# resemble-ai/flowhigh

Hardware: NVIDIA B200
Metric: 48kHz audio-sec/sec (whole job) (higher is better)
Workload: dtype fp16

## Files before the change

flowhigh_b200/_lib.py:

```python
from __future__ import annotations

import ctypes as C
import os
from typing import Optional

from .build import lib_path

_i, _i64, _f, _p = C.c_int, C.c_int64, C.c_float, C.c_void_p


class TcConvArgs(C.Structure):
    _fields_ = [
        ("a", _p), ("a_batch", _i64), ("a_chunk", _i64), ("a_row0", _i),
        ("w", _p), ("bias", _p), ("res", _p), ("out", _p),
        ("out_batch", _i64), ("out_chunk", _i64), ("out_row", _i64),
        ("res_batch", _i64), ("res_chunk", _i64), ("res_row", _i64),
        ("out_is_16", _i), ("res_is_16", _i),
        ("alpha", _f), ("beta_res", _f),
        ("accumulate", _i), ("geglu", _i),
        ("B", _i), ("L", _i), ("Cin", _i), ("Cout", _i),
        ("ntaps", _i), ("P", _i),
        ("tap_off", C.POINTER(_i)),
        ("bn", _i),
        ("fp16", _i),
# ... 30 lines not shown
    "fh_dwconv_gelu_res_f32": (_i, [_p, _p, _p, _p, _i, _i, _i, _i, _p]),
    "fh_dwconv_f32": (_i, [_p, _p, _p, _p, _i, _i, _i, _i, _p]),
    "fh_layernorm_f32": (_i, [_p, _p, _p, _p, _i, _i64, _i, _i, _f, _p]),
    "fh_gelu_f32": (_i, [_p, _p, _i, _i64, _i, _i, _p]),
    "fh_rmsnorm_f32": (_i, [_p, _p, _p, _p, _i, _i64, _i, _i, _p]),
    "fh_qknorm_rope_f32": (_i, [_p, _p, _p, _p, _p, _p, _p, _i, _i, _i, _i, _p]),
    "fh_attention_f32": (_i, [_p, _p, _p, _p, _i, _i64, _i, _i, _i, _i, _f, _p]),
    "fh_qknorm_rope_split": (_i, [_p, _p, _p, _p, _p, _p, _p, _p, _p, _i, _i, _i, _i, _f, _i, _p]),
    "fh_attention_tc": (_i, [_p, _p, _p, _p, _p, _p, _i, _i64, _i, _i, _i, _i, _i, _p]),
    "fh_attention_tc5_operand_elems": (_i64, [_i, _i, _i, _i]),
    "fh_qknorm_rope_tiles": (_i, [_p, _p, _p, _p, _p, _p, _p, _i, _i, _i, _i, _f, _i, _p]),
    "fh_attention_tc5": (_i, [_p, _p, _p, _p, _i, _i64, _i, _i, _i, _i, _i, _p]),
    "fh_geglu_f32": (_i, [_p, _p, _i, _i64, _i, _i, _i, _p]),
    "fh_axpby_f32": (_i, [_p, _p, _f, _f, _p, _i64, _p]),
    "fh_rk_lincomb_f32": (_i, [_p, _p, _i64, _i, C.POINTER(_f), _p, _i64, _p]),
    "fh_rk_scaled_sumsq_f32": (_i, [_p, _p, _p, _f, _f, _i, _i64, _p, _p]),
    "fh_broadcast_row_f32": (_i, [_p, _p, _i64, _i, _p]),
    "fh_mel_cutoff_f32": (_i, [_p, _p, _i, _i, _i, _f, _p]),
    "fh_mel_splice_f32": (_i, [_p, _p, _p, _p, _i, _i, _i, _p]),
    "fh_conv1d_taps_f32": (_i, [_p, _p, _p, _p, _p, _f, _f, _i, _p, _i, _i, _i, _i, _i, _i, _p]),
    "fh_snake_aa_f32": (_i, [_p, _p, _p, _p, _p, _i, _i, _i, _p]),
    "fh_convpost_tanh_f32": (_i, [_p, _p, _f, _p, _i, _i, _i, _p]),
    "fh_transpose_f32": (_i, [_p, _p, _i, _i, _i, _p]),
    "fh_cast_f32_16": (_i, [_p, _p, _i64, _i, _p]),
    "fh_cast_f32_16_split": (_i, [_p, _p, _i64, _i, _i64, _i64, _i, _i, _p]),
    "fh_sum_cast_f32": (_i, [_p, _p, _p, _p, _p, _p, _i64, _i, _p]),
    "fh_tc_conv": (_i, [C.POINTER(TcConvArgs), _p]),
    "fh_tc_packed_weight_bytes": (_i64, [_i, _i, _i, _i, _i]),
    "fh_to_chunked_16": (_i, [_p, _i64, _i64, _i64, _p, _i64, _i64, _i, _i, _i, _i, _i, _p]),
    "fh_to_chunked_16_split": (_i, [_p, _i64, _i64, _i64, _p, _i64, _i64, _i, _i, _i, _i, _i, _p]),
    "fh_snake_aa_chunked_split": (_i, [_p, _p, _p, _p, _p, _i64, _i64, _i64, _i, _i, _i, _i, _p]),
    "fh_snake_aa_chunked": (_i, [_p, _p, _p, _p, _p, _i64, _i64, _i, _i, _i, _i, _i, _p]),
    "fh_snake_aa_chunked_h": (_i, [_p, _p, _p, _p, _p, _i64, _i64, _i, _i, _i, _i, _p]),
    "fh_snakepost_convpost_tanh": (_i, [_p, _i64, _i64, _i, _p, _p, _p, _p, _f, _p, _i, _i, _i, _p]),
    "fh_convpost_tanh_chunked": (_i, [_p, _i64, _i64, _i, _p, _f, _p, _i, _i, _i, _p]),
}

_lib: Optional[C.CDLL] = None


class FlowHighNativeError(RuntimeError):
    pass


def load(build_if_missing: bool = True) -> C.CDLL:
    global _lib
    if _lib is not None:
        return _lib
    path = lib_path()
    if build_if_missing and os.environ.get("FLOWHIGH_B200_NO_BUILD") != "1":
        try:
            from .build import build
            path = build()
        except Exception as e:
            if not os.path.exists(path):
                raise FlowHighNativeError(f"libflowhigh_b200.so is missing and cannot be built: {e}") from e
    if not os.path.exists(path):
        raise FlowHighNativeError(
            f"{path} not found: run `python -m flowhigh_b200.build` (nvcc, sm_100a). There is no fallback path.")
    lib = C.CDLL(path)
    for name, (res, args) in SIGNATURES.items():
        fn = getattr(lib, name)
        fn.restype = res
        fn.argtypes = args
    _lib = lib
    return lib
# ... 16 lines not shown
```

flowhigh_b200/csrc/snake_mma.cuh:

```cuda
#pragma once
#include <cuda_fp16.h>
#include "snake_worker.cuh"
#ifndef FH_SNAKE_K8
#define FH_SNAKE_K8 1
#endif

namespace fh {

template <int NB>
struct SnakeMmaGeom {
  static constexpr int kWarps = 4;
  static constexpr int kSeg = 8 * NB;
  static constexpr int kWarpRows = 2 * kSeg;
  static constexpr int kRows = kWarps * kWarpRows;
  static constexpr int kHalo = 8;
  static constexpr int kXRows = kRows + 2 * kHalo;
  static constexpr int kXBytes = kXRows * 32;
  static constexpr int kWarpYBytes = kWarpRows * 16;
  static constexpr int smem_bytes(bool in16, bool split_out = false, int wbuf = 2) {
    return wbuf * (in16 ? kXBytes / 2 : kXBytes) + (split_out ? 4 : 2) * kWarps * kWarpYBytes + 128;
  }
};

__device__ __forceinline__ uint32_t sm_pack(float lo, float hi) {
// ... 213 lines not shown
      }
    }
  }
  if (edge) {
    __syncwarp();
    for (int w = lane; w < 48; w += 32) {
      const int c = w & 7, o = w >> 3;
      const int qq = o < 3 ? o : L - 6 + o;
      if (qq >= q0 && qq < q0 + G::kWarpRows && qq < L && (o < 3 || qq >= 3)) {
        const int cc = ch * 8 + c;
        const float alv = 2.0f * __ldg(sn_a + cc), hib = 0.5f * __ldg(sn_inv_b + cc);
        float acc = hib;
        for (int k = 0; k < 12; ++k) {
          const int m = min(max(2 * qq + k - 5, 0), 2 * L - 1);
          const int ihi = (m + 5) >> 1;
          float u = 0.f;
          for (int t6 = 0; t6 < 6; ++t6) {
            const int i = ihi - t6;
            const int ic = min(max(i, 0), L - 1);
            const int xi = (ic - q0 + G::kHalo) * 8 + c;
            const float xv = IN16 ? __half2float(reinterpret_cast<const __half*>(xw)[xi]) : xw[xi];
            u = fmaf(2.0f * __ldg(sn_filt + (m + 5 - 2 * i)), xv, u);
          }
          acc = fmaf(__ldg(sn_filt + k), u - hib * __cosf(alv * u), acc);
        }
        const __half hv = __float2half_rn(acc);
        *reinterpret_cast<__half*>(yt + (size_t)(qq - q0) * 16 + 2 * c) = hv;
        if (SPLIT_OUT) *reinterpret_cast<__half*>(yt_lo + (size_t)(qq - q0) * 16 + 2 * c) = __float2half_rn(acc - __half2float(hv));
      }
    }
  }
}

template <bool SPLIT_X, bool SPLIT_F, int NB, bool IN16 = false, bool SPLIT_OUT = false, int WBUF = 2>
__device__ __forceinline__ void snake_mma_cta(const SnakeParams& S, unsigned char* smem, int tid, int cta, int nctas) {
  using G = SnakeMmaGeom<NB>;
  const int lane = tid & 31, warp = tid >> 5;
  constexpr int kXB = IN16 ? G::kXBytes / 2 : G::kXBytes;
  float* xs0 = reinterpret_cast<float*>(smem);
  float* xs1 = reinterpret_cast<float*>(smem + (WBUF - 1) * kXB);
  constexpr int kImg = SPLIT_OUT ? 2 : 1;
  unsigned char* ys0 = smem + WBUF * kXB + warp * 2 * kImg * G::kWarpYBytes;
  unsigned char* ctl = smem + WBUF * kXB + 2 * kImg * G::kWarps * G::kWarpYBytes;
  const uint32_t bar0 = sw_u32(ctl);
  int* released = reinterpret_cast<int*>(ctl + 16);
  float* s_taps = reinterpret_cast<float*>(ctl + 32);
  if (tid == 0) {
    asm volatile("mbarrier.init.shared::cta.b64 [%0], 1;" ::"r"(bar0) : "memory");
    asm volatile("mbarrier.init.shared::cta.b64 [%0], 1;" ::"r"(bar0 + 8) : "memory");
    asm volatile("fence.mbarrier_init.release.cluster;" ::: "memory");
    released[0] = released[1] = 0;
  }
  if (tid < 4) snake_mma_make_taps<SPLIT_F>(S.filt, s_taps, tid);
  for (int i = tid; i < WBUF * kXB / 16; i += 32 * G::kWarps) reinterpret_cast<float4*>(smem)[i] = make_float4(0.f, 0.f, 0.f, 0.f);
  asm volatile("fence.proxy.async.shared::cta;" ::: "memory");
  __syncthreads();
  const int rows_per_chunk = (int)(S.chunk_stride >> 3);
  const int d_tile = nctas % S.ntile, d_rest = nctas / S.ntile;
  const int d_ch = d_rest % S.nchunk, d_b = d_rest / S.nchunk;
  auto advance = [&](int& tile, int& ch, int& b) {
    tile += d_tile;
    ch += d_ch;
    b += d_b;
    if (tile >= S.ntile) tile -= S.ntile, ++ch;
    if (ch >= S.nchunk) ch -= S.nchunk, ++b;
  };
  auto issue = [&](int tile, int ch, int b, int buf) {
    const int r_first = S.row0 + tile * G::kRows - G::kHalo;
    int nrows = rows_per_chunk - r_first;
    nrows = nrows < G::kXRows ? nrows : G::kXRows;
    const long long eoff = (long long)b * S.batch_stride + (long long)ch * S.chunk_stride + (long long)r_first * 8;
    const void* src = IN16 ? (const void*)((const unsigned short*)S.x + eoff) : (const void*)(S.x + eoff);
    const uint32_t bytes = (uint32_t)nrows * (IN16 ? 16u : 32u);
    const uint32_t bar = bar0 + 8 * buf;
    asm volatile("mbarrier.arrive.expect_tx.shared::cta.b64 _, [%0], %1;" ::"r"(bar), "r"(bytes) : "memory");
    asm volatile("cp.async.bulk.shared::cluster.global.mbarrier::complete_tx::bytes [%0], [%1], %2, [%3];" ::"r"(
                     sw_u32(buf ? xs1 : xs0)),
                 "l"(src), "r"(bytes), "r"(bar)
                 : "memory");
  };

  SnakeFrags F;
  snake_mma_frags<IN16>(s_taps, lane, F);
  Guard16 guard;
  int item = cta;
  int tile = item % S.ntile, ch = (item / S.ntile) % S.nchunk, b = (item / S.ntile) / S.nchunk;
  int tile_f = tile, ch_f = ch, b_f = b;
  if (tid == 0 && item < S.total) issue(tile, ch, b, 0);
  advance(tile_f, ch_f, b_f);
  if (WBUF == 2) {
    if (tid == 0 && item + nctas < S.total) issue(tile_f, ch_f, b_f, 1);
    advance(tile_f, ch_f, b_f);
  }
  int buf = 0, ybuf = 0;
  uint32_t ph0 = 0, ph1 = 0;
  const int ssA = warp * G::kWarpRows;
  for (; item < S.total; item += nctas, advance(tile, ch, b), advance(tile_f, ch_f, b_f)) {
    const int qt = tile * G::kRows;
    const bool edge = (tile == 0) || (qt + G::kRows + G::kHalo > S.L);
    const bool active = qt + ssA < S.L;
    sw_mbar_wait(bar0 + 8 * buf, buf ? ph1 : ph0);
    if (buf) ph1 ^= 1; else ph0 ^= 1;
    float* xt = buf ? xs1 : xs0;
    unsigned char* yt = ys0 + (size_t)ybuf * kImg * G::kWarpYBytes;
    if (active) {
      float* xw = reinterpret_cast<float*>(reinterpret_cast<unsigned char*>(xt) + (size_t)ssA * (IN16 ? 16 : 32));
      snake_mma_unit<SPLIT_X, SPLIT_F, NB, IN16, SPLIT_OUT>(F, xw, yt, qt + ssA, S.L, ch, S.a, S.inv_b, S.filt, edge, -ssA,
                                                            G::kXRows - ssA, lane, guard, yt + G::kWarpYBytes);
    }
    asm volatile("fence.proxy.async.shared::cta;" ::: "memory");
    if (lane == 0) asm volatile("cp.async.bulk.wait_group.read 0;" ::: "memory");
    __syncwarp();
    if (lane == 0) {
      if (active) {
        const int nrows = min(G::kWarpRows, S.L - qt - ssA);
        const unsigned short* dst = (const unsigned short*)S.y + (long long)b * S.y_batch_stride +
                                    (long long)ch * S.chunk_stride + (long long)(S.row0 + qt + ssA) * 8;
        asm volatile("cp.async.bulk.global.shared::cta.bulk_group [%0], [%1], %2;" ::"l"(dst), "r"(sw_u32(yt)),
                     "r"((uint32_t)nrows * 16u)
                     : "memory");
        if (SPLIT_OUT)
          asm volatile("cp.async.bulk.global.shared::cta.bulk_group [%0], [%1], %2;" ::"l"(dst + S.lo_offset),
                       "r"(sw_u32(yt + G::kWarpYBytes)), "r"((uint32_t)nrows * 16u)
                       : "memory");
        asm volatile("cp.async.bulk.commit_group;" ::: "memory");
      }
      __threadfence_block();
      if (atomicAdd(&released[buf], 1) == G::kWarps - 1) {
        released[buf] = 0;
        __threadfence_block();
        if (item + WBUF * nctas < S.total) {
          asm volatile("fence.proxy.async.shared::cta;" ::: "memory");
          issue(tile_f, ch_f, b_f, buf);
        }
      }
    }
    if (WBUF == 2) buf ^= 1;
    ybuf ^= 1;
  }
  if (lane == 0) asm volatile("cp.async.bulk.wait_group.read 0;" ::: "memory");
  guard.commit(S.status, 1);
}

}
```

flowhigh_b200/csrc/snake_worker.cuh:

```cuda
#pragma once
#include "common.cuh"

namespace fh {

struct SnakeParams {
  const float* x;
  void* y;
  const float* a;
  const float* inv_b;
  const float* filt;
  long long batch_stride, chunk_stride;
  long long y_batch_stride;
  long long lo_offset;
  int row0, nchunk, L, ntile, total;
  int fp16;
  unsigned int* status;
};

template <int R>
struct SnakeGeom {
  static constexpr int kRows = R * 32;
  static constexpr int kXRows = kRows + 10;
  static constexpr int kXBytes = kXRows * 32;
  static constexpr int kYBytes = kRows * 16;
  static constexpr int kSmemBytes = ((2 * kXBytes + kYBytes + 16 + 127) / 128) * 128;
};

__device__ __forceinline__ float2 sw_ffma2(float2 a, float2 b, float2 c) {
  unsigned long long ra = *reinterpret_cast<unsigned long long*>(&a), rb = *reinterpret_cast<unsigned long long*>(&b),
                     rc = *reinterpret_cast<unsigned long long*>(&c), rd;
  asm("fma.rn.f32x2 %0, %1, %2, %3;" : "=l"(rd) : "l"(ra), "l"(rb), "l"(rc));
  return *reinterpret_cast<float2*>(&rd);
}
__device__ __forceinline__ float2 sw_fmul2(float2 a, float2 b) {
  unsigned long long ra = *reinterpret_cast<unsigned long long*>(&a), rb = *reinterpret_cast<unsigned long long*>(&b), rd;
  asm("mul.rn.f32x2 %0, %1, %2;" : "=l"(rd) : "l"(ra), "l"(rb));
  return *reinterpret_cast<float2*>(&rd);
}
__device__ __forceinline__ uint32_t sw_u32(const void* p) { return (uint32_t)__cvta_generic_to_shared(p); }
__device__ __forceinline__ void sw_mbar_wait(uint32_t bar, uint32_t parity) {
  uint32_t ok = 0;
  const long long t0 = clock64();
  while (!ok) {
    asm volatile(
        "{\n\t.reg .pred p;\n\t"
        "mbarrier.try_wait.parity.shared::cta.b64 p, [%1], %2, %3;\n\t"
        "selp.b32 %0, 1, 0, p;\n\t}"
        : "=r"(ok)
        : "r"(bar), "r"(parity), "r"(2000u)
// ... 155 lines not shown
```

flowhigh_b200/csrc/vocoder_tc.cu:

```cuda
#include <stdlib.h>
#include "common.cuh"
#include "snake_worker.cuh"
#include "snake_mma.cuh"

namespace {

constexpr int PR = 17;

template <int OUT_KIND, bool BULK_OUT>
__global__ void __launch_bounds__(128, 4) snake_aa_chunked_tma_kernel(const __grid_constant__ fh::SnakeParams S) {
  extern __shared__ __align__(128) unsigned char snake_smem[];
  fh::snake_worker<OUT_KIND, BULK_OUT, PR>(S, snake_smem, threadIdx.x, blockIdx.x, gridDim.x, 0);
}

template <int MODE, int NB, int MINB, bool IN16, bool SPLIT_OUT, int WBUF>
__global__ void __launch_bounds__(128, MINB) snake_aa_mma_kernel(const __grid_constant__ fh::SnakeParams S) {
  extern __shared__ __align__(128) unsigned char snake_smem[];
  fh::snake_mma_cta<(MODE & 1) != 0, (MODE & 2) != 0, NB, IN16, SPLIT_OUT, WBUF>(S, snake_smem, threadIdx.x, blockIdx.x,
                                                                                 gridDim.x);
}

template <int MODE, int NB, int MINB, bool IN16 = false, bool SPLIT_OUT = false, int WBUF = 2>
void launch_snake_mma(fh::SnakeParams sp, int B, int C, int L, int sms, cudaStream_t stream) {
  using G = fh::SnakeMmaGeom<NB>;
  static int smem_set[64] = {0};
  fh::ensure_dyn_smem(snake_aa_mma_kernel<MODE, NB, MINB, IN16, SPLIT_OUT, WBUF>, G::smem_bytes(IN16, SPLIT_OUT, WBUF), smem_set);
  sp.ntile = (L + G::kRows - 1) / G::kRows;
  const long long total = (long long)sp.ntile * (C / 8) * B;
  sp.total = (int)total;
  const int grid = (int)(total < (long long)sms * MINB ? total : (long long)sms * MINB);
  snake_aa_mma_kernel<MODE, NB, MINB, IN16, SPLIT_OUT, WBUF><<<grid, 128, G::smem_bytes(IN16, SPLIT_OUT, WBUF), stream>>>(sp);
}

constexpr int kCpT = 256;
__global__ void __launch_bounds__(kCpT) convpost_tanh_chunked_kernel(const float* __restrict__ x, long long batch_stride,
                                                                     long long chunk_stride, int row0,
                                                                     const float* __restrict__ w, float bias,
                                                                     float* __restrict__ y, int C, int L) {
  extern __shared__ __align__(16) float cp_smem[];
  const int nchunk = C >> 3;
  float* s_w = cp_smem;
  float* tile = cp_smem + ((C * 7 + 3) & ~3);
  const int b = blockIdx.y, t0 = blockIdx.x * kCpT;
  for (int i = threadIdx.x; i < C * 7; i += kCpT) s_w[i] = __ldg(w + i);
  const float* xb = x + (long long)b * batch_stride;
  const int rows = kCpT + 6;
  for (int i = threadIdx.x; i < nchunk * rows * 2; i += kCpT) {
    const int h = i & 1, r = (i >> 1) % rows, ch = (i >> 1) / rows;
    const int t = t0 - 3 + r;
    float4 v = make_float4(0.f, 0.f, 0.f, 0.f);
    if (t >= 0 && t < L) v = __ldg(reinterpret_cast<const float4*>(xb + (long long)ch * chunk_stride + (long long)(row0 + t) * 8) + h);
    reinterpret_cast<float4*>(tile)[i] = v;
  }
  __syncthreads();
  const int t = t0 + threadIdx.x;
  if (t >= L) return;
  float acc = bias;
  for (int ch = 0; ch < nchunk; ++ch) {
    const float* tp = tile + ((size_t)ch * rows + threadIdx.x) * 8;
    const float* wp = s_w + ch * 56;
#pragma unroll
    for (int j = 0; j < 7; ++j) {
      const float4 v0 = *reinterpret_cast<const float4*>(tp + j * 8), v1 = *reinterpret_cast<const float4*>(tp + j * 8 + 4);
      acc = fmaf(wp[j], v0.x, acc);
// ... 113 lines not shown
    for (int r = 0; r < 10; ++r) {
      const float4 v0 = *reinterpret_cast<const float4*>(tp + sp_row_off(o + r));
      const float4 v1 = *reinterpret_cast<const float4*>(tp + sp_row_off(o + r) + 16);
      const float v[8] = {v0.x, v0.y, v0.z, v0.w, v1.x, v1.y, v1.z, v1.w};
#pragma unroll
      for (int oo = 0; oo < 4; ++oo) {
        const int j = r - oo;
        if (j >= 0 && j < 7) {
#pragma unroll
          for (int c = 0; c < 8; ++c) acc[oo] = fmaf(wr[c * 7 + j], v[c], acc[oo]);
        }
      }
    }
  }
  float* yp = y + (long long)b * L + t0 + o;
  if (t0 + o + 3 < L && ((((long long)b * L + t0 + o) & 3) == 0)) {
    *reinterpret_cast<float4*>(yp) = make_float4(tanhf(acc[0]), tanhf(acc[1]), tanhf(acc[2]), tanhf(acc[3]));
  } else {
#pragma unroll
    for (int oo = 0; oo < 4; ++oo)
      if (t0 + o + oo < L) yp[oo] = tanhf(acc[oo]);
  }
}

}

extern "C" __attribute__((visibility("default"))) int fh_snake_aa_chunked(
    const float* x, void* y, const float* a, const float* inv_b, const float* filt, int64_t batch_stride,
    int64_t chunk_stride, int row0, int B, int C, int L, int out_kind, void* stream) {
  FH_REQUIRE(B > 0 && C > 0 && (C % 8) == 0 && L > 0, FH_ERR_BAD_SHAPE, "fh_snake_aa_chunked: C must be a multiple of 8");
  FH_REQUIRE(out_kind >= 0 && out_kind <= 2, FH_ERR_BAD_SHAPE, "fh_snake_aa_chunked: out_kind must be 0 (fp32), 1 (bf16), 2 (fp16)");
  FH_REQUIRE(((uintptr_t)x % 16) == 0 && (batch_stride % 8) == 0 && (chunk_stride % 8) == 0, FH_ERR_BAD_ALIGN,
             "fh_snake_aa_chunked: x must be 16-byte aligned and strides multiples of 8");
  static int mma_mode = -2;
  if (mma_mode == -2) {
    const char* e = getenv("FH_SNAKE_MMA");
    mma_mode = e ? atoi(e) : 0;
    if (mma_mode < -1 || mma_mode > 3) mma_mode = 0;
  }
  const bool use_mma = out_kind == 2 && mma_mode >= 0 && row0 >= fh::SnakeMmaGeom<8>::kHalo;
  constexpr int kTileRows = fh::SnakeGeom<PR>::kRows;
  const int ntile = (L + kTileRows - 1) / kTileRows;
  const long long total = (long long)ntile * (C / 8) * B;
  FH_REQUIRE(total <= 2147483647LL && row0 >= 5, FH_ERR_BAD_SHAPE, "fh_snake_aa_chunked: needs a left halo of >= 5 rows");
  const int sms = fh::dev_sms();
  static int per_sm = 0;
  if (!per_sm) {
    const char* e = getenv("FH_SNAKE_CTAS_PER_SM");
    per_sm = e ? atoi(e) : 4;
    if (per_sm < 1 || per_sm > 4) per_sm = 4;
  }
  const int grid = (int)(total < (long long)sms * per_sm ? total : (long long)sms * per_sm);
  static int bulk = -1;
  if (bulk < 0) {
    const char* e = getenv("FH_SNAKE_BULK");
    bulk = e ? atoi(e) : 1;
  }
  fh::SnakeParams sp;
  sp.x = x, sp.y = y, sp.a = a, sp.inv_b = inv_b, sp.filt = filt;
  sp.batch_stride = batch_stride, sp.chunk_stride = chunk_stride, sp.y_batch_stride = batch_stride, sp.lo_offset = 0;
  sp.row0 = row0, sp.nchunk = C / 8, sp.L = L, sp.ntile = ntile, sp.total = (int)total, sp.fp16 = out_kind == 2;
  sp.status = fh::status_word();
  if (use_mma) {
    FH_REQUIRE((long long)((L + 511) / 512) * (C / 8) * B <= 2147483647LL, FH_ERR_BAD_SHAPE, "fh_snake_aa_chunked: too many work items");
    cudaStream_t cs = (cudaStream_t)stream;
    static int nb16 = -1;
    if (nb16 < 0) {
      const char* e = getenv("FH_SNAKE_NB");
      nb16 = (e && atoi(e) == 8) ? 0 : 1;
    }
    static int wbuf1 = -1;
    if (wbuf1 < 0) {
      const char* e = getenv("FH_SNAKE_WBUF");
      wbuf1 = (e && atoi(e) == 1) ? 1 : 0;
    }
    if (mma_mode == 0 && nb16 && wbuf1) launch_snake_mma<0, 16, 3, false, false, 1>(sp, B, C, L, sms, cs);
    else if (mma_mode == 0 && nb16) launch_snake_mma<0, 16, 2>(sp, B, C, L, sms, cs);
    else if (mma_mode == 0) launch_snake_mma<0, 8, 4>(sp, B, C, L, sms, cs);
    else if (mma_mode == 3) launch_snake_mma<3, 8, 4>(sp, B, C, L, sms, cs);
    else launch_snake_mma<1, 8, 4>(sp, B, C, L, sms, cs);
    return fh::check_launch("fh_snake_aa_chunked");
  }
  constexpr int kSmem = fh::SnakeGeom<PR>::kSmemBytes;
#define FH_SNAKE_LAUNCH(KIND, BULK) snake_aa_chunked_tma_kernel<KIND, BULK><<<grid, 128, kSmem, (cudaStream_t)stream>>>(sp)
  if (out_kind == 0) FH_SNAKE_LAUNCH(0, false);
  else if (out_kind == 1 && bulk) FH_SNAKE_LAUNCH(1, true);
  else if (out_kind == 1) FH_SNAKE_LAUNCH(1, false);
  else if (bulk) FH_SNAKE_LAUNCH(2, true);
  else FH_SNAKE_LAUNCH(2, false);
#undef FH_SNAKE_LAUNCH
  return fh::check_launch("fh_snake_aa_chunked");
}

extern "C" __attribute__((visibility("default"))) int fh_snake_aa_chunked_split(
    const float* x, void* y, const float* a, const float* inv_b, const float* filt, int64_t x_batch_stride,
    int64_t y_batch_stride, int64_t chunk_stride, int row0, int B, int C, int L, void* stream) {
  FH_REQUIRE(B > 0 && C > 0 && (C % 8) == 0 && L > 0, FH_ERR_BAD_SHAPE, "fh_snake_aa_chunked_split: C must be a multiple of 8");
  FH_REQUIRE(((uintptr_t)x % 16) == 0 && ((uintptr_t)y % 16) == 0 && (x_batch_stride % 8) == 0 && (y_batch_stride % 8) == 0 &&
                 (chunk_stride % 8) == 0,
             FH_ERR_BAD_ALIGN, "fh_snake_aa_chunked_split: buffers must be 16-byte aligned and strides multiples of 8");
  FH_REQUIRE(row0 >= fh::SnakeMmaGeom<8>::kHalo, FH_ERR_BAD_SHAPE, "fh_snake_aa_chunked_split: needs a left halo of >= 8 rows");
  FH_REQUIRE((long long)((L + 511) / 512) * (C / 8) * B <= 2147483647LL, FH_ERR_BAD_SHAPE,
             "fh_snake_aa_chunked_split: too many work items");
  fh::SnakeParams sp;
  sp.x = x, sp.y = y, sp.a = a, sp.inv_b = inv_b, sp.filt = filt;
  sp.batch_stride = x_batch_stride, sp.chunk_stride = chunk_stride, sp.y_batch_stride = y_batch_stride;
  sp.lo_offset = (int64_t)(C / 8) * chunk_stride;
  sp.row0 = row0, sp.nchunk = C / 8, sp.L = L, sp.ntile = 0, sp.total = 0, sp.fp16 = 1;
  sp.status = fh::status_word();
  launch_snake_mma<1, 8, 3, false, true>(sp, B, C, L, fh::dev_sms(), (cudaStream_t)stream);
  return fh::check_launch("fh_snake_aa_chunked_split");
}

extern "C" __attribute__((visibility("default"))) int fh_snake_aa_chunked_h(
    const void* x16, void* y, const float* a, const float* inv_b, const float* filt, int64_t batch_stride,
    int64_t chunk_stride, int row0, int B, int C, int L, void* stream) {
  FH_REQUIRE(B > 0 && C > 0 && (C % 8) == 0 && L > 0, FH_ERR_BAD_SHAPE, "fh_snake_aa_chunked_h: C must be a multiple of 8");
  FH_REQUIRE(((uintptr_t)x16 % 16) == 0 && ((uintptr_t)y % 16) == 0 && (batch_stride % 8) == 0 && (chunk_stride % 8) == 0,
             FH_ERR_BAD_ALIGN, "fh_snake_aa_chunked_h: buffers must be 16-byte aligned and strides multiples of 8");
  FH_REQUIRE(row0 >= fh::SnakeMmaGeom<8>::kHalo, FH_ERR_BAD_SHAPE, "fh_snake_aa_chunked_h: needs a left halo of >= 8 rows");
  FH_REQUIRE((long long)((L + 511) / 512) * (C / 8) * B <= 2147483647LL, FH_ERR_BAD_SHAPE,
             "fh_snake_aa_chunked_h: too many work items");
  const int sms = fh::dev_sms();
  fh::SnakeParams sp;
// ... 56 lines not shown
```

flowhigh_b200/engine.py:

```python
from __future__ import annotations

import collections
import contextlib
from os import environ as _environ
_os_environ_get = _environ.get
import ctypes as C
import math
from typing import Dict, Optional

import numpy as np
import torch

from . import _lib, packing, tables
from .config import BackboneConfig, MelConfig, VocoderConfig
from .weights import FH, VOC

HALO = 32


def _ptr(t: Optional[torch.Tensor]) -> Optional[int]:
    return None if t is None else t.data_ptr()


class _TcWeight:
# ... 110 lines not shown
        t = self._bufs.get(key)
        self._buf_last[key] = self._buf_epoch
        if t is not None:
            self._bufs.move_to_end(key)
        if t is None:
            need = int(np.prod(key[1], dtype=np.int64)) * torch.empty((), dtype=dtype).element_size()
            if self._buf_bytes + need > self._buf_cap:
                self._evict_for(need)
            t = (torch.zeros if zero else torch.empty)(key[1], dtype=dtype, device=self.device)
            self._bufs[key] = t
            self._buf_bytes += need
            if not torch.cuda.is_current_stream_capturing():
                torch.cuda.current_stream(self.device).synchronize()
        if self._touch_log is not None:
            self._touch_log[id(t)] = t
        return t

    def _chk(self, *tensors):
        for t in tensors:
            if t is None:
                continue
            if t.device != self.device or t.dtype != torch.float32 or not t.is_contiguous():
                raise ValueError(f"engine tensors must be contiguous fp32 on {self.device} "
                                 f"(got {t.dtype}, {t.device}, contiguous={t.is_contiguous()})")

    def _call(self, name, *args, work=None):
        if self.profile is None:
            _lib.check(getattr(self.lib, name)(*args), name)
            return
        if work is None and name == "fh_snake_aa_chunked":
            work = {"bytes": float(args[8] * args[9] * args[10]) * (8.0 if args[11] == 0 else 6.0)}
        if work is None and name == "fh_snake_aa_chunked_h":
            work = {"bytes": float(args[8] * args[9] * args[10]) * 4.0, "tag": "fh_snake_aa_chunked"}
        if work is None and name == "fh_rmsnorm_f32":
            work = {"bytes": float(args[6] * args[7]) * (8.0 if args[4] == 0 else 6.0)}
        self._profile_cool()
        e0, e1 = torch.cuda.Event(enable_timing=True), torch.cuda.Event(enable_timing=True)
        e0.record(torch.cuda.current_stream(self.device))
        _lib.check(getattr(self.lib, name)(*args), name)
        e1.record(torch.cuda.current_stream(self.device))
        self.profile.append((name, e0, e1, work or {}))

    def _profile_cool(self):
        if self._cool_ms > 0.0:
            import time
            torch.cuda.synchronize(self.device)
            time.sleep(self._cool_ms * 1e-3)

    def start_profile(self):
        self.profile = []

    def stop_profile(self):
        torch.cuda.synchronize(self.device)
        agg = {}
        for name, e0, e1, work in self.profile or []:
            key = work.get("tag", name)
            d = agg.setdefault(key, {"ms": 0.0, "launches": 0, "flops": 0.0, "bytes": 0.0})
            d["ms"] += e0.elapsed_time(e1)
            d["launches"] += 1
            d["flops"] += work.get("flops", 0.0)
            d["bytes"] += work.get("bytes", 0.0)
        self.profile = None
        return agg

    def _mk_f32(self, tconv: packing.TappedConv) -> _F32Weight:
        r = _F32Weight()
# ... 86 lines not shown
        return a, ib, filt_up.contiguous()

    def _prep_vocoder(self):
        sd, v = self.sd, self.vcfg
        mk = (lambda t, residual=False, **kw: self._mk_tc(t, split=self.split, two_cta=self._pair_wins(
            t.cout, t.ntaps, t.P, residual), **kw)) if self.tc else (lambda t, residual=False, **kw: self._mk_f32(t))
        pad = (lambda c: packing.round_up(c, 8)) if self.tc else (lambda c: c)
        self.cpad = pad
        V = {}
        C0 = v.upsample_initial_channel
        kw = dict(cin_pad=pad(v.num_mels), cout_pad=pad(C0)) if self.tc else {}
        V["conv_pre"] = mk(packing.conv1d_taps(sd[VOC + "conv_pre.weight"], sd[VOC + "conv_pre.bias"]), **kw)
        nk = v.num_kernels
        for s, (u, k) in enumerate(zip(v.upsample_rates, v.upsample_kernel_sizes)):
            cin, cout = C0 // (2 ** s), v.stage_channels(s)
            kw = dict(cin_pad=pad(cin), cout_pad=pad(cout)) if self.tc else {}
            V[f"up{s}"] = mk(packing.conv_transpose1d_taps(sd[VOC + f"ups.{s}.0.weight"], sd[VOC + f"ups.{s}.0.bias"], u),
                             **kw)
            for j, (kk, dil) in enumerate(zip(v.resblock_kernel_sizes, v.resblock_dilation_sizes)):
                p = VOC + f"resblocks.{s * nk + j}."
                kw = dict(cin_pad=pad(cout), cout_pad=pad(cout)) if self.tc else {}
                for i, d in enumerate(dil):
                    if v.resblock == "1":
                        V[f"r{s}.{j}.c1.{i}"] = mk(packing.conv1d_taps(sd[p + f"convs1.{i}.weight"],
                                                                       sd[p + f"convs1.{i}.bias"], d), **kw)
                        V[f"r{s}.{j}.c2.{i}"] = mk(packing.conv1d_taps(sd[p + f"convs2.{i}.weight"],
                                                                       sd[p + f"convs2.{i}.bias"], 1), residual=True, **kw)
                        V[f"r{s}.{j}.a1.{i}"] = self._snake_params(p + f"activations.{2 * i}.", pad(cout))
                        V[f"r{s}.{j}.a2.{i}"] = self._snake_params(p + f"activations.{2 * i + 1}.", pad(cout))
                    else:
                        V[f"r{s}.{j}.c1.{i}"] = mk(packing.conv1d_taps(sd[p + f"convs.{i}.weight"],
                                                                       sd[p + f"convs.{i}.bias"], d), residual=True, **kw)
                        V[f"r{s}.{j}.a1.{i}"] = self._snake_params(p + f"activations.{i}.", pad(cout))
        clast = v.stage_channels(v.num_stages - 1)
        V["post_act"] = self._snake_params(VOC + "activation_post.", pad(clast))
        wpost = torch.zeros(pad(clast), 7, device=self.device)
        wpost[:clast] = sd[VOC + "conv_post.weight"][0]
        V["post_w"] = wpost.contiguous()
        V["post_b"] = float(sd[VOC + "conv_post.bias"].item())
        self.voc = V

    def resample_normalise(self, x: torch.Tensor, sr_in: int, sr_out: int = 48000, method: str = "scipy") -> torch.Tensor:
        self._chk(x)
        B, T_in = x.shape
        if method not in ("scipy", "soxr_hq"):
            raise ValueError(f"unknown resampling method {method!r} (scipy|soxr_hq)")
        plan = tables.resample_plan(sr_in, sr_out) if method == "scipy" else tables.resample_plan_soxr_hq(sr_in, sr_out)
        absmax = self.buf("rs_absmax", (B,), torch.int32)
        self._call("fh_fill_u32", absmax.data_ptr(), 0, B, self.stream)
        if plan is None:
            y, T_out = x, T_in
            self._call("fh_absmax_f32", y.data_ptr(), absmax.data_ptr(), B, T_out, self.stream)
        else:
            h, up, down, npp, npr = plan
            key = (sr_in, sr_out, method)
            if key not in self._resample_taps:
                self._resample_taps[key] = torch.from_numpy(h).to(self.device)
            hd = self._resample_taps[key]
            T_out = tables.resample_out_len(T_in, up, down)
            y = self.buf("rs_y", (B, T_out), zero=False)
            self._call("fh_resample_poly_f32", x.data_ptr(), y.data_ptr(), hd.data_ptr(), absmax.data_ptr(), B, T_in,
                       T_out, hd.numel(), up, down, npp, npr, self.stream,
                       work={"bytes": 4.0 * B * (T_in + T_out), "flops": 2.0 * B * T_out * (hd.numel() // up + 1)})
        cond = torch.empty((B, T_out), dtype=torch.float32, device=self.device)
        self._call("fh_scale_by_absmax_f32", y.data_ptr(), cond.data_ptr(), absmax.data_ptr(), 1.0, B, T_out, self.stream,
                   work={"bytes": 8.0 * B * T_out})
# ... 502 lines not shown
        B, N, nm = mel.shape
        bf, f32 = self.h16, torch.float32
        _cb = self._cbuf
        self_cbuf = lambda name, *a: _cb(name + tag, *a)
        melc, mcs, mbs = self_cbuf("vt_mel", B, nm, N, bf)
        self._call("fh_to_chunked_16", mel.data_ptr(), N * nm, 1, nm, melc.data_ptr(), mbs, mcs, HALO, B, nm, N, self.fp16, st)
        C0 = self.cpad(v.upsample_initial_channel)
        xb, xcs, xbs = self_cbuf("vt_pre", B, C0, N, bf)
        self._tc_conv(V["conv_pre"], melc, mbs, mcs, HALO, xb[HALO * 8:], (xbs, xcs, 8), 1, B, N)
        L = N
        nk = v.num_kernels
        a_in, a_cs, a_bs = xb, xcs, xbs
        par = (self.branch_streams and B <= self.branch_streams_max_batch and started_event is None and nk > 1)
        main = torch.cuda.current_stream(self.device)
        if par:
            while len(self._branch_streams) < nk:
                self._branch_streams.append(torch.cuda.Stream(self.device))
        for s, u in enumerate(v.upsample_rates):
            ch = self.cpad(v.stage_channels(s))
            Lo = L * u
            X, cs, bs = self_cbuf(f"vt_X{s}", B, ch, Lo, f32)
            o = HALO * 8
            strides = (bs, cs, 8)
            self._tc_conv(V[f"up{s}"], a_in, a_bs, a_cs, HALO, X[o:], strides, 0, B, L)
            L = Lo
            fuse = self.fuse_snake and ch <= 128 and all(V[f"r{s}.{j}.c1.0"].bn >= ch for j in range(nk))
            if par:
                ev_up = torch.cuda.Event()
                ev_up.record(main)
            outs = []
            fuse_cast = (not par and nk > 1 and s + 1 < v.num_stages and _os_environ_get("FH_FUSE_CAST", "1") != "0")
            if fuse_cast:
                XBf, _, _ = self_cbuf(f"vt_XB{s}", B, ch, Lo, bf)
            for j, dil in enumerate(v.resblock_dilation_sizes):
                bt = f"_{j}" if par else ""
                XJ, _, _ = self_cbuf(f"vt_XJ{s}{bt}", B, ch, Lo, f32)
                y16 = (self.y16 or fuse) and v.resblock == "1"
                Y, _, _ = self_cbuf(f"vt_Y{s}{bt}" + ("h" if y16 else ""), B, ch, Lo, bf if y16 else f32)
                A = None if fuse else self_cbuf(f"vt_A{s}{bt}", B, ch, Lo, bf)[0]
                XSj, _, _ = self_cbuf(f"vt_XS{s}_{j}" if par else f"vt_XS{s}", B, ch, Lo, f32)
                outs.append(XSj)
                ctx = torch.cuda.stream(self._branch_streams[j]) if par else contextlib.nullcontext()
                if par:
                    self._branch_streams[j].wait_event(ev_up)
                with ctx:
                    st = self.stream
                    cur = X
                    for i in range(len(dil)):
                        last = i == len(dil) - 1
                        sn1 = V[f"r{s}.{j}.a1.{i}"]
                        if not fuse:
                            self._call("fh_snake_aa_chunked", cur.data_ptr(), A.data_ptr(), sn1[0].data_ptr(), sn1[1].data_ptr(),
                                       sn1[2].data_ptr(), bs, cs, HALO, B, ch, L, self.k16, st)
                        if started_event is not None:
                            started_event.record(torch.cuda.current_stream(self.device))
                            started_event = None
                        fa = dict(xf=cur, snake=sn1) if fuse else {}
                        if v.resblock == "1":
                            self._tc_conv(V[f"r{s}.{j}.c1.{i}"], None if fuse else A, bs, cs, HALO, Y[o:], strides,
                                          1 if y16 else 0, B, L, **fa)
                            sn2 = V[f"r{s}.{j}.a2.{i}"]
                            if fuse:
                                pass
                            elif y16:
                                self._call("fh_snake_aa_chunked_h", Y.data_ptr(), A.data_ptr(), sn2[0].data_ptr(),
                                           sn2[1].data_ptr(), sn2[2].data_ptr(), bs, cs, HALO, B, ch, L, st)
                            else:
                                self._call("fh_snake_aa_chunked", Y.data_ptr(), A.data_ptr(), sn2[0].data_ptr(),
                                           sn2[1].data_ptr(), sn2[2].data_ptr(), bs, cs, HALO, B, ch, L, self.k16, st)
                            fa = dict(xf=Y, snake=sn2, x16=True) if fuse else {}
                            conv = V[f"r{s}.{j}.c2.{i}"]
                        else:
                            conv = V[f"r{s}.{j}.c1.{i}"]
                        src = None if fuse else A
                        if last and fuse_cast and j == nk - 1:
                            self._tc_conv(conv, src, bs, cs, HALO, XBf[o:], strides, 1, B, L, res=cur[o:], res_strides=strides,
                                          alpha=1.0 / nk, beta=1.0 / nk, accumulate=True, acc_src=XSj[o:], **fa)
                        elif last:
                            self._tc_conv(conv, src, bs, cs, HALO, XSj[o:], strides, 0, B, L, res=cur[o:], res_strides=strides,
                                          alpha=1.0 / nk, beta=1.0 / nk, accumulate=(j > 0 and not par), **fa)
                        else:
                            self._tc_conv(conv, src, bs, cs, HALO, XJ[o:], strides, 0, B, L, res=cur[o:], res_strides=strides,
                                          beta=1.0, **fa)
                            cur = XJ
                    if par:
                        done = torch.cuda.Event()
                        done.record(self._branch_streams[j])
                        main.wait_event(done)
            st = self.stream
            XS, _, _ = self_cbuf(f"vt_XS{s}", B, ch, Lo, f32)
            if par:
                if len(outs) > 4:
                    raise ValueError("at most 4 resblock kernel sizes per stage")
                ptrs = [t_.data_ptr() for t_ in outs] + [None] * (4 - len(outs))
            if s + 1 < v.num_stages:
                XB, _, _ = self_cbuf(f"vt_XB{s}", B, ch, L, bf)
                if par:
                    self._call("fh_sum_cast_f32", *ptrs, None, XB.data_ptr(), B * bs, self.fp16, st)
                elif not fuse_cast:
                    self._call("fh_cast_f32_16", XS.data_ptr(), XB.data_ptr(), B * bs, self.fp16, st)
                a_in, a_cs, a_bs = XB, cs, bs
            elif par:
                self._call("fh_sum_cast_f32", *ptrs, XS.data_ptr(), None, B * bs, self.fp16, st)
        self._post(XS, bs, cs, B, ch, L, wave, self_cbuf)

    def _post(self, XS, bs, cs, B, ch, L, wave, cbuf):
        V, st = self.voc, self.stream
# ... 104 lines not shown
```

include/flowhigh_b200.h:

```cpp
#ifndef FLOWHIGH_B200_H
#define FLOWHIGH_B200_H

#include <stdint.h>

#ifdef __cplusplus
extern "C" {
#endif

#define FH_OK 0
#define FH_ERR_BAD_SHAPE (-1)
#define FH_ERR_BAD_ALIGN (-2)
#define FH_ERR_UNSUPPORTED_CFG (-3)
#define FH_ERR_CUDA (-4)

int fh_version(void);
const char* fh_last_error_string(void);
int64_t fh_launch_count(void);
int fh_set_status_word(uint32_t* status);
int fh_set_debug_word(uint32_t* word);

int fh_resample_poly_f32(const float* x, float* y, const float* h, uint32_t* absmax_bits,
                         int B, int T_in, int T_out, int ntaps, int up, int down,
                         int n_pre_pad, int n_pre_remove, void* stream);
int fh_scale_by_absmax_f32(const float* x, float* y, const uint32_t* absmax_bits, float scale,
// ... 92 lines not shown
  int64_t res_batch, res_chunk, res_row;
  int out_is_16, res_is_16;
  float alpha, beta_res;
  int accumulate;
  int geglu;
  int B, L, Cin, Cout;
  int ntaps, P;
  const int* tap_off;
  int bn;
  int fp16;
  const void* x_f32;
  const float* sn_a;
  const float* sn_inv_b;
  const float* sn_filt;
  int act;
  const float* acc_src;
  int x_is_16;
  int two_cta;
} fh_tc_conv_args;
int fh_tc_conv(const fh_tc_conv_args* args, void* stream);
int64_t fh_tc_packed_weight_bytes(int Cin, int Cout, int ntaps, int P, int bn);

int fh_to_chunked_16(const float* src, int64_t src_batch, int64_t src_c, int64_t src_t,
                     void* dst, int64_t dst_batch, int64_t dst_chunk, int dst_row0,
                     int B, int C, int L, int fp16, void* stream);
int fh_to_chunked_16_split(const float* src, int64_t src_batch, int64_t src_c, int64_t src_t,
                           void* dst, int64_t dst_batch, int64_t dst_chunk, int dst_row0,
                           int B, int C, int L, int fp16, void* stream);
int fh_snake_aa_chunked(const float* x, void* y, const float* a, const float* inv_b, const float* filt,
                        int64_t batch_stride, int64_t chunk_stride, int row0, int B, int C, int L,
                        int out_kind, void* stream);
int fh_snake_aa_chunked_h(const void* x16, void* y, const float* a, const float* inv_b, const float* filt,
                          int64_t batch_stride, int64_t chunk_stride, int row0, int B, int C, int L, void* stream);
int fh_snake_aa_chunked_split(const float* x, void* y, const float* a, const float* inv_b, const float* filt,
                              int64_t x_batch_stride, int64_t y_batch_stride, int64_t chunk_stride, int row0,
                              int B, int C, int L, void* stream);
int fh_convpost_tanh_chunked(const float* x, int64_t batch_stride, int64_t chunk_stride, int row0,
                             const float* w, float bias, float* y, int B, int C, int L, void* stream);

int fh_snakepost_convpost_tanh(const float* x, int64_t batch_stride, int64_t chunk_stride, int row0,
                               const float* a, const float* inv_b, const float* filt, const float* w, float bias,
                               float* y, int B, int C, int L, void* stream);

#ifdef __cplusplus
}
#endif
#endif
```

Measured before the change: 2256.

## Fuse first snake activations of all resblock branches into one multi-set kernel

When the resblock branches share the same input and anti-alias filter, a new multi-set snake kernel loads each input tile once and writes snake outputs for up to three parameter sets (one per branch) into separate buffers. Each branch's first conv then reads its precomputed buffer instead of launching its own snake kernel. This cuts repeated reads of the fp32 input and the per-branch launches, at the cost of extra per-branch staging buffers and a longer per-tile loop in the kernel.

```diff
diff --git a/flowhigh_b200/_lib.py b/flowhigh_b200/_lib.py
--- a/flowhigh_b200/_lib.py
+++ b/flowhigh_b200/_lib.py
@@ -86,6 +86,7 @@
     "fh_snake_aa_chunked_split": (_i, [_p, _p, _p, _p, _p, _i64, _i64, _i64, _i, _i, _i, _i, _p]),
     "fh_snake_aa_chunked": (_i, [_p, _p, _p, _p, _p, _i64, _i64, _i, _i, _i, _i, _i, _p]),
     "fh_snake_aa_chunked_h": (_i, [_p, _p, _p, _p, _p, _i64, _i64, _i, _i, _i, _i, _p]),
+    "fh_snake_aa_chunked_multi": (_i, [_p, _i, _p, _p, _p, _p, _p, _p, _p, _p, _p, _p, _i64, _i64, _i, _i, _i, _i, _p]),
     "fh_snakepost_convpost_tanh": (_i, [_p, _i64, _i64, _i, _p, _p, _p, _p, _f, _p, _i, _i, _i, _p]),
     "fh_convpost_tanh_chunked": (_i, [_p, _i64, _i64, _i, _p, _f, _p, _i, _i, _i, _p]),
 }
diff --git a/flowhigh_b200/csrc/snake_mma.cuh b/flowhigh_b200/csrc/snake_mma.cuh
--- a/flowhigh_b200/csrc/snake_mma.cuh
+++ b/flowhigh_b200/csrc/snake_mma.cuh
@@ -269,7 +269,7 @@
   }
 }
 
-template <bool SPLIT_X, bool SPLIT_F, int NB, bool IN16 = false, bool SPLIT_OUT = false, int WBUF = 2>
+template <bool SPLIT_X, bool SPLIT_F, int NB, bool IN16 = false, bool SPLIT_OUT = false, int WBUF = 2, bool MULTI = false>
 __device__ __forceinline__ void snake_mma_cta(const SnakeParams& S, unsigned char* smem, int tid, int cta, int nctas) {
   using G = SnakeMmaGeom<NB>;
   const int lane = tid & 31, warp = tid >> 5;
@@ -332,6 +332,7 @@
   int buf = 0, ybuf = 0;
   uint32_t ph0 = 0, ph1 = 0;
   const int ssA = warp * G::kWarpRows;
+  const int nsets = MULTI ? S.nsets : 1;
   for (; item < S.total; item += nctas, advance(tile, ch, b), advance(tile_f, ch_f, b_f)) {
     const int qt = tile * G::kRows;
     const bool edge = (tile == 0) || (qt + G::kRows + G::kHalo > S.L);
@@ -339,19 +340,21 @@
     sw_mbar_wait(bar0 + 8 * buf, buf ? ph1 : ph0);
     if (buf) ph1 ^= 1; else ph0 ^= 1;
     float* xt = buf ? xs1 : xs0;
-    unsigned char* yt = ys0 + (size_t)ybuf * kImg * G::kWarpYBytes;
-    if (active) {
-      float* xw = reinterpret_cast<float*>(reinterpret_cast<unsigned char*>(xt) + (size_t)ssA * (IN16 ? 16 : 32));
-      snake_mma_unit<SPLIT_X, SPLIT_F, NB, IN16, SPLIT_OUT>(F, xw, yt, qt + ssA, S.L, ch, S.a, S.inv_b, S.filt, edge, -ssA,
-                                                            G::kXRows - ssA, lane, guard, yt + G::kWarpYBytes);
-    }
-    asm volatile("fence.proxy.async.shared::cta;" ::: "memory");
-    if (lane == 0) asm volatile("cp.async.bulk.wait_group.read 0;" ::: "memory");
-    __syncwarp();
-    if (lane == 0) {
+    float* xw = reinterpret_cast<float*>(reinterpret_cast<unsigned char*>(xt) + (size_t)ssA * (IN16 ? 16 : 32));
+#pragma unroll 1
+    for (int k = 0; k < nsets; ++k) {
+      unsigned char* yt = ys0 + (size_t)ybuf * kImg * G::kWarpYBytes;
       if (active) {
+        snake_mma_unit<SPLIT_X, SPLIT_F, NB, IN16, SPLIT_OUT>(F, xw, yt, qt + ssA, S.L, ch, k ? S.more_a[k - 1] : S.a,
+                                                              k ? S.more_inv_b[k - 1] : S.inv_b, S.filt, edge, -ssA,
+                                                              G::kXRows - ssA, lane, guard, yt + G::kWarpYBytes);
+      }
+      asm volatile("fence.proxy.async.shared::cta;" ::: "memory");
+      if (lane == 0) asm volatile("cp.async.bulk.wait_group.read 0;" ::: "memory");
+      __syncwarp();
+      if (lane == 0 && active) {
         const int nrows = min(G::kWarpRows, S.L - qt - ssA);
-        const unsigned short* dst = (const unsigned short*)S.y + (long long)b * S.y_batch_stride +
+        const unsigned short* dst = (const unsigned short*)(k ? S.more_y[k - 1] : S.y) + (long long)b * S.y_batch_stride +
                                     (long long)ch * S.chunk_stride + (long long)(S.row0 + qt + ssA) * 8;
         asm volatile("cp.async.bulk.global.shared::cta.bulk_group [%0], [%1], %2;" ::"l"(dst), "r"(sw_u32(yt)),
                      "r"((uint32_t)nrows * 16u)
@@ -362,6 +365,9 @@
                        : "memory");
         asm volatile("cp.async.bulk.commit_group;" ::: "memory");
       }
+      ybuf ^= 1;
+    }
+    if (lane == 0) {
       __threadfence_block();
       if (atomicAdd(&released[buf], 1) == G::kWarps - 1) {
         released[buf] = 0;
@@ -373,7 +379,6 @@
       }
     }
     if (WBUF == 2) buf ^= 1;
-    ybuf ^= 1;
   }
   if (lane == 0) asm volatile("cp.async.bulk.wait_group.read 0;" ::: "memory");
   guard.commit(S.status, 1);
diff --git a/flowhigh_b200/csrc/snake_worker.cuh b/flowhigh_b200/csrc/snake_worker.cuh
--- a/flowhigh_b200/csrc/snake_worker.cuh
+++ b/flowhigh_b200/csrc/snake_worker.cuh
@@ -15,6 +15,10 @@
   int row0, nchunk, L, ntile, total;
   int fp16;
   unsigned int* status;
+  int nsets = 1;
+  const float* more_a[2] = {nullptr, nullptr};
+  const float* more_inv_b[2] = {nullptr, nullptr};
+  void* more_y[2] = {nullptr, nullptr};
 };
 
 template <int R>
diff --git a/flowhigh_b200/csrc/vocoder_tc.cu b/flowhigh_b200/csrc/vocoder_tc.cu
--- a/flowhigh_b200/csrc/vocoder_tc.cu
+++ b/flowhigh_b200/csrc/vocoder_tc.cu
@@ -13,23 +13,35 @@
   fh::snake_worker<OUT_KIND, BULK_OUT, PR>(S, snake_smem, threadIdx.x, blockIdx.x, gridDim.x, 0);
 }
 
-template <int MODE, int NB, int MINB, bool IN16, bool SPLIT_OUT, int WBUF>
+template <int MODE, int NB, int MINB, bool IN16, bool SPLIT_OUT, int WBUF, bool MULTI>
 __global__ void __launch_bounds__(128, MINB) snake_aa_mma_kernel(const __grid_constant__ fh::SnakeParams S) {
   extern __shared__ __align__(128) unsigned char snake_smem[];
-  fh::snake_mma_cta<(MODE & 1) != 0, (MODE & 2) != 0, NB, IN16, SPLIT_OUT, WBUF>(S, snake_smem, threadIdx.x, blockIdx.x,
-                                                                                 gridDim.x);
-}
-
-template <int MODE, int NB, int MINB, bool IN16 = false, bool SPLIT_OUT = false, int WBUF = 2>
+  fh::snake_mma_cta<(MODE & 1) != 0, (MODE & 2) != 0, NB, IN16, SPLIT_OUT, WBUF, MULTI>(S, snake_smem, threadIdx.x,
+                                                                                        blockIdx.x, gridDim.x);
+}
+
+template <int MODE, int NB, int MINB, bool IN16 = false, bool SPLIT_OUT = false, int WBUF = 2, bool MULTI = false>
 void launch_snake_mma(fh::SnakeParams sp, int B, int C, int L, int sms, cudaStream_t stream) {
   using G = fh::SnakeMmaGeom<NB>;
   static int smem_set[64] = {0};
-  fh::ensure_dyn_smem(snake_aa_mma_kernel<MODE, NB, MINB, IN16, SPLIT_OUT, WBUF>, G::smem_bytes(IN16, SPLIT_OUT, WBUF), smem_set);
+  fh::ensure_dyn_smem(snake_aa_mma_kernel<MODE, NB, MINB, IN16, SPLIT_OUT, WBUF, MULTI>, G::smem_bytes(IN16, SPLIT_OUT, WBUF),
+                      smem_set);
   sp.ntile = (L + G::kRows - 1) / G::kRows;
   const long long total = (long long)sp.ntile * (C / 8) * B;
   sp.total = (int)total;
   const int grid = (int)(total < (long long)sms * MINB ? total : (long long)sms * MINB);
-  snake_aa_mma_kernel<MODE, NB, MINB, IN16, SPLIT_OUT, WBUF><<<grid, 128, G::smem_bytes(IN16, SPLIT_OUT, WBUF), stream>>>(sp);
+  snake_aa_mma_kernel<MODE, NB, MINB, IN16, SPLIT_OUT, WBUF, MULTI>
+      <<<grid, 128, G::smem_bytes(IN16, SPLIT_OUT, WBUF), stream>>>(sp);
+}
+
+int snake_mma_mode() {
+  static int mode = -2;
+  if (mode == -2) {
+    const char* e = getenv("FH_SNAKE_MMA");
+    mode = e ? atoi(e) : 0;
+    if (mode < -1 || mode > 3) mode = 0;
+  }
+  return mode;
 }
 
 constexpr int kCpT = 256;
@@ -209,12 +221,7 @@
   FH_REQUIRE(out_kind >= 0 && out_kind <= 2, FH_ERR_BAD_SHAPE, "fh_snake_aa_chunked: out_kind must be 0 (fp32), 1 (bf16), 2 (fp16)");
   FH_REQUIRE(((uintptr_t)x % 16) == 0 && (batch_stride % 8) == 0 && (chunk_stride % 8) == 0, FH_ERR_BAD_ALIGN,
              "fh_snake_aa_chunked: x must be 16-byte aligned and strides multiples of 8");
-  static int mma_mode = -2;
-  if (mma_mode == -2) {
-    const char* e = getenv("FH_SNAKE_MMA");
-    mma_mode = e ? atoi(e) : 0;
-    if (mma_mode < -1 || mma_mode > 3) mma_mode = 0;
-  }
+  const int mma_mode = snake_mma_mode();
   const bool use_mma = out_kind == 2 && mma_mode >= 0 && row0 >= fh::SnakeMmaGeom<8>::kHalo;
   constexpr int kTileRows = fh::SnakeGeom<PR>::kRows;
   const int ntile = (L + kTileRows - 1) / kTileRows;
@@ -267,6 +274,41 @@
   else FH_SNAKE_LAUNCH(2, false);
 #undef FH_SNAKE_LAUNCH
   return fh::check_launch("fh_snake_aa_chunked");
+}
+
+extern "C" __attribute__((visibility("default"))) int fh_snake_aa_chunked_multi(
+    const float* x, int nk, void* y0, const float* a0, const float* inv_b0, void* y1, const float* a1, const float* inv_b1,
+    void* y2, const float* a2, const float* inv_b2, const float* filt, int64_t batch_stride, int64_t chunk_stride, int row0,
+    int B, int C, int L, void* stream) {
+  FH_REQUIRE(nk >= 1 && nk <= 3, FH_ERR_BAD_SHAPE, "fh_snake_aa_chunked_multi: nk must be 1, 2 or 3");
+  void* ys[3] = {y0, y1, y2};
+  const float* as[3] = {a0, a1, a2};
+  const float* ibs[3] = {inv_b0, inv_b1, inv_b2};
+  for (int k = 0; k < nk; ++k)
+    FH_REQUIRE(ys[k] && as[k] && ibs[k] && ((uintptr_t)ys[k] % 16) == 0, FH_ERR_BAD_ALIGN,
+               "fh_snake_aa_chunked_multi: set %d needs a, inv_b and a 16-byte aligned y", k);
+  if (snake_mma_mode() != 0) {
+    for (int k = 0; k < nk; ++k) {
+      const int rc = fh_snake_aa_chunked(x, ys[k], as[k], ibs[k], filt, batch_stride, chunk_stride, row0, B, C, L, 2, stream);
+      if (rc != 0) return rc;
+    }
+    return 0;
+  }
+  FH_REQUIRE(B > 0 && C > 0 && (C % 8) == 0 && L > 0, FH_ERR_BAD_SHAPE, "fh_snake_aa_chunked_multi: C must be a multiple of 8");
+  FH_REQUIRE(((uintptr_t)x % 16) == 0 && (batch_stride % 8) == 0 && (chunk_stride % 8) == 0, FH_ERR_BAD_ALIGN,
+             "fh_snake_aa_chunked_multi: x must be 16-byte aligned and strides multiples of 8");
+  FH_REQUIRE(row0 >= fh::SnakeMmaGeom<16>::kHalo, FH_ERR_BAD_SHAPE, "fh_snake_aa_chunked_multi: needs a left halo of >= 8 rows");
+  FH_REQUIRE((long long)((L + 511) / 512) * (C / 8) * B <= 2147483647LL, FH_ERR_BAD_SHAPE,
+             "fh_snake_aa_chunked_multi: too many work items");
+  fh::SnakeParams sp;
+  sp.x = x, sp.y = y0, sp.a = a0, sp.inv_b = inv_b0, sp.filt = filt;
+  sp.batch_stride = batch_stride, sp.chunk_stride = chunk_stride, sp.y_batch_stride = batch_stride, sp.lo_offset = 0;
+  sp.row0 = row0, sp.nchunk = C / 8, sp.L = L, sp.ntile = 0, sp.total = 0, sp.fp16 = 1;
+  sp.status = fh::status_word();
+  sp.nsets = nk;
+  for (int k = 1; k < nk; ++k) sp.more_y[k - 1] = ys[k], sp.more_a[k - 1] = as[k], sp.more_inv_b[k - 1] = ibs[k];
+  launch_snake_mma<0, 16, 2, false, false, 2, true>(sp, B, C, L, fh::dev_sms(), (cudaStream_t)stream);
+  return fh::check_launch("fh_snake_aa_chunked_multi");
 }
 
 extern "C" __attribute__((visibility("default"))) int fh_snake_aa_chunked_split(
diff --git a/flowhigh_b200/engine.py b/flowhigh_b200/engine.py
--- a/flowhigh_b200/engine.py
+++ b/flowhigh_b200/engine.py
@@ -166,6 +166,8 @@
             work = {"bytes": float(args[8] * args[9] * args[10]) * (8.0 if args[11] == 0 else 6.0)}
         if work is None and name == "fh_snake_aa_chunked_h":
             work = {"bytes": float(args[8] * args[9] * args[10]) * 4.0, "tag": "fh_snake_aa_chunked"}
+        if work is None and name == "fh_snake_aa_chunked_multi":
+            work = {"bytes": float(args[15] * args[16] * args[17]) * (4.0 + 2.0 * args[1]), "tag": "fh_snake_aa_chunked"}
         if work is None and name == "fh_rmsnorm_f32":
             work = {"bytes": float(args[6] * args[7]) * (8.0 if args[4] == 0 else 6.0)}
         self._profile_cool()
@@ -318,6 +320,7 @@
                         V[f"r{s}.{j}.c1.{i}"] = mk(packing.conv1d_taps(sd[p + f"convs.{i}.weight"],
                                                                        sd[p + f"convs.{i}.bias"], d), residual=True, **kw)
                         V[f"r{s}.{j}.a1.{i}"] = self._snake_params(p + f"activations.{i}.", pad(cout))
+            V[f"r{s}.a1.0.shared_filt"] = all(torch.equal(V[f"r{s}.{j}.a1.0"][2], V[f"r{s}.0.a1.0"][2]) for j in range(nk))
         clast = v.stage_channels(v.num_stages - 1)
         V["post_act"] = self._snake_params(VOC + "activation_post.", pad(clast))
         wpost = torch.zeros(pad(clast), 7, device=self.device)
@@ -886,6 +889,18 @@
             fuse_cast = (not par and nk > 1 and s + 1 < v.num_stages and _os_environ_get("FH_FUSE_CAST", "1") != "0")
             if fuse_cast:
                 XBf, _, _ = self_cbuf(f"vt_XB{s}", B, ch, Lo, bf)
+            multi = (not par and not fuse and 1 < nk <= 3 and self.k16 == 2 and V[f"r{s}.a1.0.shared_filt"])
+            if multi:
+                A0 = [self_cbuf(f"vt_A{s}" + (f"_b{j}" if j else ""), B, ch, Lo, bf)[0] for j in range(nk)]
+                sets = []
+                for j in range(3):
+                    if j < nk:
+                        a_, ib_, _ = V[f"r{s}.{j}.a1.0"]
+                        sets += [A0[j].data_ptr(), a_.data_ptr(), ib_.data_ptr()]
+                    else:
+                        sets += [None, None, None]
+                self._call("fh_snake_aa_chunked_multi", X.data_ptr(), nk, *sets, V[f"r{s}.0.a1.0"][2].data_ptr(), bs, cs,
+                           HALO, B, ch, L, self.stream)
             for j, dil in enumerate(v.resblock_dilation_sizes):
                 bt = f"_{j}" if par else ""
                 XJ, _, _ = self_cbuf(f"vt_XJ{s}{bt}", B, ch, Lo, f32)
@@ -903,7 +918,9 @@
                     for i in range(len(dil)):
                         last = i == len(dil) - 1
                         sn1 = V[f"r{s}.{j}.a1.{i}"]
-                        if not fuse:
+                        pre = multi and i == 0
+                        Ai = A0[j] if pre else A
+                        if not fuse and not pre:
                             self._call("fh_snake_aa_chunked", cur.data_ptr(), A.data_ptr(), sn1[0].data_ptr(), sn1[1].data_ptr(),
                                        sn1[2].data_ptr(), bs, cs, HALO, B, ch, L, self.k16, st)
                         if started_event is not None:
@@ -911,7 +928,7 @@
                             started_event = None
                         fa = dict(xf=cur, snake=sn1) if fuse else {}
                         if v.resblock == "1":
-                            self._tc_conv(V[f"r{s}.{j}.c1.{i}"], None if fuse else A, bs, cs, HALO, Y[o:], strides,
+                            self._tc_conv(V[f"r{s}.{j}.c1.{i}"], None if fuse else Ai, bs, cs, HALO, Y[o:], strides,
                                           1 if y16 else 0, B, L, **fa)
                             sn2 = V[f"r{s}.{j}.a2.{i}"]
                             if fuse:
@@ -924,9 +941,10 @@
                                            sn2[1].data_ptr(), sn2[2].data_ptr(), bs, cs, HALO, B, ch, L, self.k16, st)
                             fa = dict(xf=Y, snake=sn2, x16=True) if fuse else {}
                             conv = V[f"r{s}.{j}.c2.{i}"]
+                            src = None if fuse else A
                         else:
                             conv = V[f"r{s}.{j}.c1.{i}"]
-                        src = None if fuse else A
+                            src = None if fuse else Ai
                         if last and fuse_cast and j == nk - 1:
                             self._tc_conv(conv, src, bs, cs, HALO, XBf[o:], strides, 1, B, L, res=cur[o:], res_strides=strides,
                                           alpha=1.0 / nk, beta=1.0 / nk, accumulate=True, acc_src=XSj[o:], **fa)
diff --git a/include/flowhigh_b200.h b/include/flowhigh_b200.h
--- a/include/flowhigh_b200.h
+++ b/include/flowhigh_b200.h
@@ -148,6 +148,10 @@
                         int out_kind, void* stream);
 int fh_snake_aa_chunked_h(const void* x16, void* y, const float* a, const float* inv_b, const float* filt,
                           int64_t batch_stride, int64_t chunk_stride, int row0, int B, int C, int L, void* stream);
+int fh_snake_aa_chunked_multi(const float* x, int nk, void* y0, const float* a0, const float* inv_b0,
+                              void* y1, const float* a1, const float* inv_b1, void* y2, const float* a2,
+                              const float* inv_b2, const float* filt, int64_t batch_stride, int64_t chunk_stride,
+                              int row0, int B, int C, int L, void* stream);
 int fh_snake_aa_chunked_split(const float* x, void* y, const float* a, const float* inv_b, const float* filt,
                               int64_t x_batch_stride, int64_t y_batch_stride, int64_t chunk_stride, int row0,
                               int B, int C, int L, void* stream);
```

Result: no change. 2267 (median of 6 runs) (+0.5%).
